# nonl4331/raytracing-rust

Measured on AMD Instinct MI355X. Metric: Msamples/s on rtweekend1.ssml 1920x1080x1024spp, higher is better.
Workload: dtype f32

## Files before the change

raytracing-rust_amd/csrc/rt_lean.h:

```cpp
#pragma once

#include "rt_vec.h"

namespace rt {


RT_FN void lean_sincos(float x, float &s, float &c)
{
	const float k = rintf(x * 0.636619746685028076172f);
	float r = fmaf(-k, 1.57079637050628662109f, x);
	r = fmaf(-k, -4.37113882867379282984e-08f, r);
	r = fmaf(-k, -1.71512451000588185479e-15f, r);
	const int q = (int)k;
	const float sk = rt_sin_kernel(r), ck = rt_cos_kernel(r);
	const bool odd = (q & 1) != 0;
	const float sv = odd ? ck : sk;
	const float cv = odd ? sk : ck;
	s = (q & 2) ? -sv : sv;
	c = ((q + 1) & 2) ? -cv : cv;
}

RT_FN float lean_acos_with(float x, float sqrt_half_one_minus_abs)
{
	const bool big = fabsf(x) > 0.5f;
	const float k = rt_asin_kernel(big ? sqrt_half_one_minus_abs : x);
	const float two_k = 2.0f * k;
	return big ? (x > 0.0f ? two_k : RT_PI - two_k) : RT_FRAC_PI_2 - k;
}
RT_FN float lean_acos(float x) { return lean_acos_with(x, sqrtf(0.5f * (1.0f - fabsf(x)))); }

RT_FN float lean_atan_unit_with(float t, float q)
{
	const bool upper = t > 0.414213567972183227539f;
	const float u = upper ? q : t;
	const float z = u * u;
	float p = fmaf(8.05374449538e-2f, z, -1.38776856032e-1f);
	p = fmaf(p, z, 1.99777106478e-1f);
	p = fmaf(p, z, -3.33329491539e-1f);
	return (upper ? RT_FRAC_PI_4 : 0.0f) + fmaf(p * z, u, u);
}
template <class DivA, class DivB> RT_FN float lean_atan2_with(float y, float x, DivA div_ratio, DivB div_octant)
{
	const float ax = fabsf(x), ay = fabsf(y);
	const bool swap = ay > ax;
	const float t = div_ratio(swap ? ax : ay, swap ? ay : ax);
	const float a = lean_atan_unit_with(t, div_octant(t - 1.0f, t + 1.0f));
	float r = swap ? RT_FRAC_PI_2 - a : a;
	r = (ax == ay) ? RT_FRAC_PI_4 : r;
	r = (ax == 0.0f && ay == 0.0f) ? 0.0f : r;
	if (rt_f32_bits(x) & 0x80000000u)
		r = RT_PI - r;
	r = (rt_f32_bits(y) & 0x80000000u) ? -r : r;
	return (x != x || y != y) ? x + y : r;
}
RT_FN float lean_atan2_portable(float y, float x)
{
	return lean_atan2_with(y, x, [](float n, float d) { return n / d; }, [](float n, float d) { return n / d; });
}

RT_FN float div_by_verified(float x, float c, float rc)
{
	const float q0 = x * rc;
	const float e = fmaf(-c, q0, x);
	return fmaf(e, rc, q0);
}
constexpr float kRcpPi = 1.0f / RT_PI, kRcpTau = 1.0f / RT_TAU;

#if defined(__HIP_DEVICE_COMPILE__)

__device__ __forceinline__ float lean_rcp_refined(float d)
{
	const float r0 = __builtin_amdgcn_rcpf(d);
	const float e = __builtin_fmaf(-d, r0, 1.0f);
	return __builtin_fmaf(e, r0, r0);
}
__device__ __forceinline__ float lean_div_core(float n, float d, float r1)
{
	const float q0 = n * r1;
	const float e1 = __builtin_fmaf(-d, q0, n);
	const float q1 = __builtin_fmaf(e1, r1, q0);
	const float e2 = __builtin_fmaf(-d, q1, n);
	return __builtin_fmaf(e2, r1, q1);
}
__device__ __forceinline__ float lean_div(float n, float d) { return lean_div_core(n, d, lean_rcp_refined(d)); }
__device__ __forceinline__ float lean_div_fix(float n, float d)
{
	return __builtin_amdgcn_div_fixupf(lean_div_core(n, d, lean_rcp_refined(d)), d, n);
}
__device__ __forceinline__ float lean_inv(float d)
{
	const float r1 = lean_rcp_refined(d);
	const float e1 = __builtin_fmaf(-d, r1, 1.0f);
	const float q1 = __builtin_fmaf(e1, r1, r1);
	const float e2 = __builtin_fmaf(-d, q1, 1.0f);
	return __builtin_fmaf(e2, r1, q1);
}
__device__ __forceinline__ V3 lean_div3(V3 v, float d)
{
	const float r1 = lean_rcp_refined(d);
	return V3{lean_div_core(v.x, d, r1), lean_div_core(v.y, d, r1), lean_div_core(v.z, d, r1)};
}
__device__ __forceinline__ V3 lean_div3_fix(V3 v, float d)
{
	const float r1 = lean_rcp_refined(d);
	return V3{__builtin_amdgcn_div_fixupf(lean_div_core(v.x, d, r1), d, v.x), __builtin_amdgcn_div_fixupf(lean_div_core(v.y, d, r1), d, v.y),
	          __builtin_amdgcn_div_fixupf(lean_div_core(v.z, d, r1), d, v.z)};
}

__device__ __forceinline__ float lean_sqrt(float x)
{
	const float s = __builtin_amdgcn_sqrtf(x);
	const float s_dn = __uint_as_float(__float_as_uint(s) - 1u);
	const float s_up = __uint_as_float(__float_as_uint(s) + 1u);
	const float r_dn = __builtin_fmaf(-s_dn, s, x);
	const float r_up = __builtin_fmaf(-s_up, s, x);
	float r = (r_dn <= 0.0f) ? s_dn : s;
	r = (r_up > 0.0f) ? s_up : r;
	return r;
}
constexpr float kLeanSqrtMin = 0x1p-96f;

__device__ __forceinline__ float lean_atan2(float y, float x)
{
	return lean_atan2_with(y, x, [](float n, float d) { return n / d; }, [](float n, float d) { return lean_div_fix(n, d); });
}
__device__ __forceinline__ float lean_acos_dev(float x) { return lean_acos_with(x, lean_sqrt(0.5f * (1.0f - fabsf(x)))); }
#else
RT_FN float lean_rcp_refined(float d) { return 1.0f / d; }
RT_FN float lean_div_core(float n, float d, float) { return n / d; }
RT_FN float lean_div(float n, float d) { return n / d; }
RT_FN float lean_div_fix(float n, float d) { return n / d; }
RT_FN float lean_inv(float d) { return 1.0f / d; }
RT_FN V3 lean_div3(V3 v, float d) { return v / d; }
RT_FN V3 lean_div3_fix(V3 v, float d) { return v / d; }
RT_FN float lean_sqrt(float x) { return sqrtf(x); }
constexpr float kLeanSqrtMin = 0x1p-96f;
RT_FN float lean_atan2(float y, float x) { return lean_atan2_portable(y, x); }
RT_FN float lean_acos_dev(float x) { return lean_acos(x); }
#endif

}
```

raytracing-rust_amd/csrc/rt_render.hip:

```cpp
#include "rt_shade.h"

namespace rt {

enum : int {
	PH_GEN = 0,
	PH_NODE = 1,
	PH_LEAF = 2,
	PH_SHADE = 3,
	PH_LIGHT = 4,
	PH_SCATTER = 5,
	PH_NARROW = 6,
	PH_COUNT = 7,
	PH_NEED_PIXEL = 7,
	PH_DONE = 8,
	PH_WALK = 9
};

#ifndef RT_PQ_SPLIT
#define RT_PQ_SPLIT 1
#endif
#ifndef RT_LIGHT_PHASE_THRESHOLD
#define RT_LIGHT_PHASE_THRESHOLD 48
#endif
constexpr uint32_t kLightPhaseThreshold = RT_LIGHT_PHASE_THRESHOLD;
// ... 114 lines not shown
	unsigned long long *rays_shot;
	uint32_t *work_counter;
	uint32_t *stack_ovf;
	DevPairScene pair;
};
#if defined(__HIP_DEVICE_COMPILE__)
typedef const __attribute__((address_space(4))) RenderArgs *KArgs;
#else
typedef const RenderArgs *KArgs;
#endif

template <int METHOD, bool PRUNE, bool FINE, bool SKY_LDS, class F, bool XCHG = false>
__global__ __launch_bounds__((KernelShape<F, FINE, XCHG>::max_block), (KernelShape<F, FINE, XCHG>::waves_per_simd)) void render_kernel(const RenderArgs args_by_value)
{
	extern __shared__ __align__(16) uint32_t lds[];
	const uint32_t lane = threadIdx.x & 63u;
	const uint32_t wave = threadIdx.x >> 6;

	(void)args_by_value;
#if defined(__HIP_DEVICE_COMPILE__)
	const KArgs K = (KArgs)__builtin_amdgcn_kernarg_segment_ptr();
	auto kargs = [&]() -> KArgs {
		KArgs k = K;
		asm volatile("" : "+s"(k));
		return k;
	};
#else
	const KArgs K = &args_by_value;
	auto kargs = [&]() -> KArgs { return K; };
#endif
	DevPairScene PS = {};
	auto load_pair_scene = [&]() {
		if constexpr (F::pair) {
			const KArgs k = kargs();
#pragma unroll
			for (int i = 0; i < 3; ++i) {
				PS.c0min[i] = k->pair.c0min[i]; PS.c0max[i] = k->pair.c0max[i];
				PS.c1min[i] = k->pair.c1min[i]; PS.c1max[i] = k->pair.c1max[i];
				PS.sky_c1[i] = k->pair.sky_c1[i]; PS.sky_c2[i] = k->pair.sky_c2[i];
			}
			PS.slot0 = k->pair.slot0; PS.slot1 = k->pair.slot1; PS.rank0 = k->pair.rank0; PS.rank1 = k->pair.rank1;
#pragma unroll
			for (int i = 0; i < 4; ++i) {
				PS.sphere[0][i] = k->pair.sphere[0][i]; PS.sphere[1][i] = k->pair.sphere[1][i];
				PS.lambert[0][i] = k->pair.lambert[0][i]; PS.lambert[1][i] = k->pair.lambert[1][i];
			}
			PS.inv_radius[0] = k->pair.inv_radius[0]; PS.inv_radius[1] = k->pair.inv_radius[1];
			PS.sky_param = k->pair.sky_param;
			PS.sky_tex_type = k->pair.sky_tex_type;
		}
	};
	const DevScene S_global = K->S;
	const DevRenderParams P = K->P;
	uint32_t *const stack_ovf = K->stack_ovf;
	DevScene S = S_global;

	SkyTables T;
	uint32_t sky_words = 0;
	if (SKY_LDS) {
		const uint32_t n_rows = S.sky.res_y * (S.sky.res_x + 1u);
		const uint32_t n_all = n_rows + S.sky.res_y + 1u;
		float *lds_sky = reinterpret_cast<float *>(lds);
		for (uint32_t i = threadIdx.x; i < n_all; i += blockDim.x)
			lds_sky[i] = S.sky.row_cdf[i];
		__syncthreads();
		sky_words = (n_all + 3u) & ~3u;
		const uint32_t guide_words = (S.sky.res_y + 1u) * S.sky.guide_k / 4u;
		uint32_t *lds_guide = lds + sky_words;
		const uint32_t *src_guide = reinterpret_cast<const uint32_t *>(S.sky.guide);
		for (uint32_t i = threadIdx.x; i < guide_words; i += blockDim.x)
			lds_guide[i] = src_guide[i];
		__syncthreads();
		T.row_cdf = lds_sky;
		T.marginal_cdf = lds_sky + n_rows;
		T.guide = reinterpret_cast<const uint8_t *>(lds_guide);
		sky_words += guide_words;
	} else {
		T.row_cdf = S.sky.row_cdf;
		T.marginal_cdf = S.sky.marginal_cdf;
		T.guide = S.sky.guide;
	}
	T.guide_k = S.sky.guide_k;
	T.inv_res = reinterpret_cast<KWords>(&K->S.sky.inv_res_ok);
	uint32_t blob_words = 0;
	if (!FINE && P.scene_in_lds) {
		uint32_t *lds_blob = lds + sky_words;
		blob_words = S.blob_bytes / 4u;
		for (uint32_t i = threadIdx.x; i < blob_words; i += blockDim.x)
			lds_blob[i] = S.blob[i];
		__syncthreads();
		const char *b = reinterpret_cast<const char *>(lds_blob);
		S.nodes = reinterpret_cast<const DevNode *>(b + S.off_nodes);
		S.prims = reinterpret_cast<const DevPrim *>(b + S.off_prims);
		S.shade = reinterpret_cast<const DevShade *>(b + S.off_shade);
		S.prim_rank = reinterpret_cast<const uint32_t *>(b + S.off_rank);
		S.materials = reinterpret_cast<const DevMaterial *>(b + S.off_materials);
		S.textures = reinterpret_cast<const DevTexture *>(b + S.off_textures);
		S.lights = reinterpret_cast<const uint32_t *>(b + S.off_lights);
		S.big_leaves = reinterpret_cast<const uint2 *>(b + S.off_big_leaves);
	}
	StackMem SM;
	SM.cap = P.stack_cap;
	SM.ovf_depth = P.stack_ovf_depth;
	SM.ovf = stack_ovf;
	SM.region = lds + sky_words + blob_words;
	uint32_t *stk = SM.region + wave * (P.stack_cap * kStackStride) + lane;
	uint32_t *pool = nullptr;
	if constexpr (XCHG) {
		pool = lds + (((uint32_t)(SM.region - lds) + (blockDim.x >> 6) * (P.stack_cap * kStackStride) + 3u) & ~3u);
		if (FINE) {
			if (threadIdx.x < kXchgFineHdr)
				pool[threadIdx.x] = threadIdx.x == 3u ? kXchgShaderWaves : (threadIdx.x == 4u ? (blockDim.x >> 6) - kXchgShaderWaves : 0u);
		} else if (threadIdx.x < 4u) {
			pool[threadIdx.x] = 0u;
		}
		__syncthreads();
	}

#ifdef RT_STATS
	unsigned long long st_iters[2] = {0, 0}, st_active[2] = {0, 0}, st_gen = 0, st_hist[8] = {};
	unsigned long long st_sect[16] = {}, st_mark = wall_clock64();
	unsigned long long st_fine_clock[PH_COUNT + 1] = {};
	unsigned long long st_fine_iters[PH_COUNT] = {}, st_fine_active[PH_COUNT] = {};
#endif
	const bool sky_samplable = sky_can_sample(S);
	constexpr int known_path = F::known_materials ? kMatLambertian : kMatRead;

	int ph = PH_NEED_PIXEL;
	rt_rng rng = {1u, 2u, 3u, 4u};
	Ray ray;
	ray.o = ray.d = ray.inv = ray.shear = v3s(0.0f);
	uint32_t node = kRefDone;
	int sp = 0;
	float best_t = 0.0f;
	uint32_t best_prim = kNoPrim;
	bool any_hit = false;
	V3 thr = v3s(1.0f), outp = v3s(0.0f), mean = v3s(0.0f), wo = v3s(0.0f);
	Hit hit;
	hit.t = 0.0f;
	hit.point = hit.error = hit.normal = v3s(0.0f);
	hit.err_dot = 0.0f;
	hit.uvx = hit.uvy = 0.0f;
	hit.has_uv = hit.out = false;
	uint32_t mat = 0;
	uint32_t depth = 0, sample_local = 0, out_index = 0, pixel_index = 0, px = 0, py = 0;
	uint32_t chunk_begin = 0, chunk_n = P.spp;
	uint32_t ray_count = 0;
	unsigned long long rays_total = 0;
	bool primary = true;
	struct LightCtx {
		V3 l_wi;
		float pdf_multiplier;
		float t_limit;
		uint32_t skip;
		bool have_shadow, shadow_is_sky;
	};
	LightCtx PL;
	PL.l_wi = v3s(0.0f);
	PL.pdf_multiplier = 1.0f;
	PL.t_limit = 0.0f;
	PL.skip = kNoPrim;
	PL.have_shadow = PL.shadow_is_sky = false;

	auto begin_walk = [&](bool shadow) {
		any_hit = shadow;
		best_t = 0.0f;
		best_prim = kNoPrim;
		sp = 0;
		if (!FINE) {
			ph = PH_NODE;
			return;
		}
		if (XCHG) {
			ph = PH_WALK;
			return;
		}
		if (root_box_misses(S, ray)) {
			node = kRefDone;
			ph = shadow ? PH_SCATTER : PH_SHADE;
		} else if (S.narrow_only != 0u || !ray_is_regular(ray)) {
			ph = PH_NARROW;
		} else {
			node = S.root4_ref;
			ph = ref_is_leaf(node) ? PH_LEAF : PH_NODE;
		}
	};
	auto start_walk = [&]() {
		sp = 0;
		if (root_box_misses(S, ray)) {
			node = kRefDone;
			ph = any_hit ? PH_SCATTER : PH_SHADE;
		} else if (S.narrow_only != 0u || !ray_is_regular(ray)) {
			ph = PH_NARROW;
		} else {
			node = S.root4_ref;
			ph = ref_is_leaf(node) ? PH_LEAF : PH_NODE;
		}
	};
	auto after_step = [&]() {
		if (node == kRefDone)
			ph = any_hit ? PH_SCATTER : PH_SHADE;
		else
			ph = ref_is_leaf(node) ? PH_LEAF : PH_NODE;
	};
	auto finalize = [&](bool filter) {
		V3 c = outp;
		if (filter && (contains_nan(c) || !is_finite_any(c)))
			c = v3s(0.0f);
		if (P.sample_split > 1u) {
			mean.x += c.x;
			mean.y += c.y;
			mean.z += c.z;
		} else {
			const float i_f = (float)(sample_local + 1u);
			mean.x += (c.x - mean.x) / i_f;
			mean.y += (c.y - mean.y) / i_f;
			mean.z += (c.z - mean.z) / i_f;
		}
		rays_total += ray_count;
		sample_local += 1;
		if (sample_local == chunk_n) {
			float *const out = kargs()->out;
			out[3u * (size_t)out_index + 0u] = mean.x;
			out[3u * (size_t)out_index + 1u] = mean.y;
			out[3u * (size_t)out_index + 2u] = mean.z;
			ph = PH_NEED_PIXEL;
		} else {
			ph = PH_GEN;
		}
	};

	auto do_gen = [&]() {
		const KArgs k = kargs();
		const uint64_t seed = ((uint64_t)k->P.seed_hi << 32) | k->P.seed_lo;
		const uint64_t sample_begin = ((uint64_t)k->P.sample_begin_hi << 32) | k->P.sample_begin_lo;
		const V3 cam_o = v3(k->cam.origin[0], k->cam.origin[1], k->cam.origin[2]);
		const V3 cam_ll = v3(k->cam.lower_left[0], k->cam.lower_left[1], k->cam.lower_left[2]);
		const V3 cam_h = v3(k->cam.horizontal[0], k->cam.horizontal[1], k->cam.horizontal[2]);
		const V3 cam_v = v3(k->cam.vertical[0], k->cam.vertical[1], k->cam.vertical[2]);
		const uint32_t w1 = here_(k->P.width - 1u), h1 = here_(k->P.height - 1u);
		rt_rng_seed(&rng, seed, (uint64_t)pixel_index, sample_begin + chunk_begin + sample_local);
		RT_SECTION(15);
		const float jx = rt_rng_range_f32(&rng, 0.0f, 1.0f) + (float)px, jy = rt_rng_range_f32(&rng, 0.0f, 1.0f) + (float)py;
		float u, v;
		if (here_(k->P.w1h1_ok) != 0u) {
// ... 64 lines not shown
					else
						take = false;
					if (take) {
						best_t = t;
						best_prim = slot;
					}
				}
			}
		}
		if (occluded) {
			best_prim = 0u;
			node = kRefDone;
		} else if (sp == 0) {
			node = kRefDone;
		} else {
			--sp;
			node = SM.ovf_depth == 0u ? stack_load<false>(SM, stk, sp) : stack_load<true>(SM, stk, sp);
		}
		after_step();
	
	};

	auto do_shade = [&](auto arm_tag) {
		constexpr int arm = decltype(arm_tag)::value;
		const uint32_t prim = best_prim;
		bool finish = false;
		bool filter = true;
		Hit nh;
		uint32_t nmat;
		if (prim != kNoPrim)
			make_hit<F>(S, prim, ray, best_t, nh, nmat, PS);
		else
			make_sky_hit_lean<F>(S, nh, nmat);
		const int known_new = F::known_materials ? (prim == kNoPrim ? kMatEmit : kMatLambertian) : kMatRead;

		if (METHOD == 0) {
			ray_count += 1;
			const V3 wo_n = ray.d;
			const V3 emission = emission_of_hit<F>(S, PS, nmat, prim == kNoPrim, nh, wo_n);
			const bool exit = mat_scatter_ray<F>(S, nmat, ray, nh, rng, known_new);
			if (depth == 0) {
				outp = outp + emission;
				if (exit)
					finish = true;
			}
			if (!finish && exit) {
				outp = outp + thr * emission;
				finish = true;
			}
			if (!finish) {
				if (!mat_is_delta<F>(S, nmat))
					thr = thr * mat_eval_over_pdf<F>(S, nmat, nh, wo_n, ray.d, known_new, PS);
				else
					thr = thr * mat_eval<F>(S, nmat, nh, wo_n, ray.d, known_new, PS);
				if (depth > P.rr_threshold) {
					const float p = component_max(thr);
					if (rt_rng_f32(&rng) > p)
						finish = true;
					else
						thr = thr / p;
				}
				if (!finish) {
					depth += 1;
					if (!(depth < P.max_depth))
						finish = true;
				}
			}
		} else if (arm == 1 || (arm == 0 && primary)) {
			wo = ray.d;
			hit = nh;
			mat = nmat;
			RT_SECTION(13);
			const V3 emission = emission_of_hit<F>(S, PS, mat, prim == kNoPrim, hit, wo);
			Ray clone = ray;
			const bool exit = mat_scatter_ray<F>(S, mat, clone, hit, rng, known_new);
			outp = outp + emission;
			RT_SECTION(14);
			if (exit) {
				finish = true;
				filter = false;
			} else {
				depth = 1;
				primary = false;
				if (!(depth < P.max_depth))
					finish = true;
			}
		} else {
			const V3 m_wi = ray.d;
			const float m_pdf = mat_scattering_pdf<F>(S, mat, hit, wo, m_wi, known_path);
			const V3 le = emission_of_hit<F>(S, PS, nmat, prim == kNoPrim, hit , m_wi);
			thr = thr * mat_eval_over_pdf<F>(S, mat, hit, wo, m_wi, known_path, PS);
			RT_SECTION(11);
			if (!is_zero(le)) {
				const bool on_light = F::lights && (prim != kNoPrim) && mat_is_light(S, nmat) && !mat_is_delta<F>(S, mat);
				if (on_light || (prim == kNoPrim && sky_samplable)) {
					const uint32_t n_l = F::lights ? S.n_lights : 0u;
					const uint32_t n_choices = sky_samplable ? n_l + 1u : n_l;
					float l_pdf;
					if (prim == kNoPrim) {
						l_pdf = div_by_count(sky_pdf(S, T, m_wi), n_choices);
					} else {
						const PrimGeom g = load_prim<F>(S, prim);
						l_pdf = div_by_count(prim_scattering_pdf<F>(g, hit.point, m_wi, nh), n_choices);
					}
					const float mis_weight = power_heuristic(m_pdf, l_pdf);
					outp = outp + thr * le * mis_weight;
				} else {
					outp = outp + thr * le;
				}
			}
			RT_SECTION(12);
			if (mat_is_light<F>(S, nmat, known_new)) {
				finish = true;
			} else {
				if (depth > P.rr_threshold) {
					const float p = component_max(thr);
					if (rt_rng_f32(&rng) > p)
						finish = true;
					else
						thr = thr / p;
				}
				if (!finish) {
					wo = m_wi;
					hit = nh;
					mat = nmat;
					depth += 1;
					if (!(depth < P.max_depth))
						finish = true;
				}
			}
		}
		if (finish)
			finalize(filter);
		else if (METHOD == 1)
			ph = PH_LIGHT;
		else
			begin_walk(false);
	
	};

	auto do_light = [&](LightCtx &L, Ray &sr) {
		ray_count += 1;
		L.have_shadow = false;
		L.shadow_is_sky = false;
		L.pdf_multiplier = 1.0f;
		L.skip = kNoPrim;
		const uint32_t samplable_len = F::lights ? S.n_lights : 0u;
		bool pick_sky = false, pick_light = false;
		uint32_t light_slot = 0;
		if (samplable_len == 0u) {
			pick_sky = sky_samplable;
		} else if (!sky_samplable) {
			L.pdf_multiplier = 1.0f / (float)samplable_len;
			light_slot = rt_rng_below(&rng, samplable_len);
			pick_light = true;
		} else {
			L.pdf_multiplier = 1.0f / (float)(samplable_len + 1u);
			light_slot = rt_rng_below(&rng, samplable_len + 1u);
			if (light_slot == samplable_len)
				pick_sky = true;
			else
				pick_light = true;
		}
		const V3 shadow_origin = hit.point + 0.0001f * hit.normal;
		PrimGeom g;
		g.type = g.material = 0u;
		g.p0 = g.p1 = g.p2 = v3s(0.0f);
		if (pick_sky) {
			L.l_wi = sky_sample(S, T, rng);
			RT_SECTION(9);
			L.t_limit = __uint_as_float(0x7FC00000u);
			L.have_shadow = true;
			L.shadow_is_sky = true;
		} else if (pick_light) {
			if (S.single_light != kNoPrim) {
				L.skip = S.single_light;
				g = load_prim_uniform<F>(&S_global.prims[L.skip]);
			} else {
				L.skip = S.lights[light_slot];
				g = load_prim<F>(S, L.skip);
			}
			L.l_wi = prim_sample_visible_from_point<F>(g, hit.point, rng);
		}
		if (pick_sky || pick_light)
			sr = ray_new<F>(shadow_origin, L.l_wi);
		if (pick_light) {
			float lt;
			if (prim_t<F>(g, sr, lt) && lt > 0.0f) {
				L.t_limit = lt;
				L.have_shadow = true;
			}
		}
		if (L.have_shadow) {
			begin_walk(true);
		} else {
			best_prim = kNoPrim;
			ph = PH_SCATTER;
		}
	
	};

	auto do_scatter = [&](LightCtx &L, Ray &sr) {
		const bool occluded = best_prim != kNoPrim;
		if (L.have_shadow && !occluded) {
			bool valid = false;
			V3 le = v3s(0.0f);
			float l_pdf = 0.0f;
			if (L.shadow_is_sky) {
				le = emission_of_hit<F>(S, PS, S.sky.material, true, hit, L.l_wi);
				l_pdf = sky_pdf(S, T, L.l_wi) * L.pdf_multiplier;
				valid = true;
			} else {
				Hit lh;
				uint32_t lm;
				PrimGeom g;
				if (S.single_light != kNoPrim) {
					g = load_prim_uniform<F>(&S_global.prims[L.skip]);
					if (!F::tri || g.type == kPrimSphere) {
						make_sphere_hit_by_reciprocal(g.p0, g.p1.x, g.p1.y, sr, L.t_limit, lh);
						lm = g.material;
					} else {
						make_hit<F>(S, L.skip, sr, L.t_limit, lh, lm);
					}
				} else {
					make_hit<F>(S, L.skip, sr, L.t_limit, lh, lm);
					g = load_prim<F>(S, L.skip);
				}
				const float p = prim_scattering_pdf<F>(g, hit.point, L.l_wi, lh);
				if (p > 0.0f) {
					le = mat_get_emission<F>(S, lm, lh, L.l_wi);
					l_pdf = p * L.pdf_multiplier;
					valid = true;
				}
			}
			if (valid) {
				const float m_pdf = mat_scattering_pdf<F>(S, mat, hit, wo, L.l_wi, known_path);
				const float mis_weight = power_heuristic(l_pdf, m_pdf);
				outp = outp + thr * mat_eval<F>(S, mat, hit, wo, L.l_wi, known_path, PS) * mis_weight * le / l_pdf;
			}
		}
		RT_SECTION(10);
		ray.d = wo;
		if (mat_scatter_ray<F>(S, mat, ray, hit, rng, known_path))
			finalize(true);
		else
			begin_walk(false);
	
	};

	auto do_narrow = [&]() {
		if (any_hit) {
			best_prim = trace_any<F, PRUNE, true>(S, S_global, SM, ray, stk, PL.t_limit, PL.skip) ? 0u : kNoPrim;
			ph = PH_SCATTER;
		} else {
			trace_closest<F, PRUNE, true>(S, S_global, SM, ray, stk, best_t, best_prim);
			ph = PH_SHADE;
		}
		node = kRefDone;
		sp = 0;
	};

	auto walk_closest_pending = [&]() {
		if (ph == PH_NODE && !any_hit) {
			trace_closest<F, PRUNE>(S, S_global, SM, ray, stk, best_t, best_prim, PS);
			ph = PH_SHADE;
		}
	};
	auto walk_shadow_pending = [&](const LightCtx &L, const Ray &sr) {
		if (ph == PH_NODE && any_hit) {
			best_prim = trace_any<F, PRUNE>(S, S_global, SM, sr, stk, L.t_limit, L.skip, PS) ? 0u : kNoPrim;
			ph = PH_SCATTER;
		}
	};

	auto record_store = [&](uint32_t *rec) {
		uint4 *d = reinterpret_cast<uint4 *>(rec);
		const uint32_t fl = (hit.has_uv ? 1u : 0u) | (hit.out ? 2u : 0u) | (primary ? 4u : 0u) | (any_hit ? 8u : 0u) | (PL.have_shadow ? 16u : 0u) |
		                    (PL.shadow_is_sky ? 32u : 0u);
		d[0] = make_uint4(rng.s0, rng.s1, rng.s2, rng.s3);
		d[1] = make_uint4(__float_as_uint(thr.x), __float_as_uint(thr.y), __float_as_uint(thr.z), __float_as_uint(outp.x));
		d[2] = make_uint4(__float_as_uint(outp.y), __float_as_uint(outp.z), __float_as_uint(wo.x), __float_as_uint(wo.y));
		d[3] = make_uint4(__float_as_uint(wo.z), __float_as_uint(hit.t), __float_as_uint(hit.point.x), __float_as_uint(hit.point.y));
		d[4] = make_uint4(__float_as_uint(hit.point.z), __float_as_uint(hit.error.x), __float_as_uint(hit.error.y), __float_as_uint(hit.error.z));
		d[5] = make_uint4(__float_as_uint(hit.normal.x), __float_as_uint(hit.normal.y), __float_as_uint(hit.normal.z), __float_as_uint(hit.uvx));
		d[6] = make_uint4(__float_as_uint(hit.uvy), fl, mat, depth);
		d[7] = make_uint4(ray_count, __float_as_uint(mean.x), __float_as_uint(mean.y), __float_as_uint(mean.z));
		d[8] = make_uint4(sample_local, out_index, pixel_index, px);
		d[9] = make_uint4(py, chunk_begin, chunk_n, (uint32_t)ph);
		d[10] = make_uint4(__float_as_uint(ray.o.x), __float_as_uint(ray.o.y), __float_as_uint(ray.o.z), __float_as_uint(ray.d.x));
		d[11] = make_uint4(__float_as_uint(ray.d.y), __float_as_uint(ray.d.z), __float_as_uint(ray.inv.x), __float_as_uint(ray.inv.y));
		d[12] = make_uint4(__float_as_uint(ray.inv.z), __float_as_uint(ray.shear.x), __float_as_uint(ray.shear.y), __float_as_uint(ray.shear.z));
		d[13] = make_uint4(__float_as_uint(best_t), best_prim, __float_as_uint(PL.t_limit), PL.skip);
		d[14] = make_uint4(__float_as_uint(PL.l_wi.x), __float_as_uint(PL.l_wi.y), __float_as_uint(PL.l_wi.z), __float_as_uint(PL.pdf_multiplier));
// ... 492 lines not shown
		}
	}

	if constexpr (!FINE) {
		bool alive = true;
		uint32_t waited = 0;
		while (alive) {
			if (XCHG && METHOD == 1)
				exchange();
			acquire();
			const uint32_t n_light = (uint32_t)__popcll(__ballot(ph == PH_LIGHT));
			const uint32_t n_trace = (METHOD == 1 && RT_PQ_SPLIT) ? (uint32_t)__popcll(__ballot(ph == PH_GEN))
			                                                      : (uint32_t)__popcll(__ballot(ph == PH_GEN || ph == PH_NODE || ph == PH_LEAF || ph == PH_SHADE));
			constexpr bool kBodyAlways = RT_BODY_ALWAYS(KernelShape<F>::spheres_only);
			if (kBodyAlways) {
				alive = (n_light + n_trace != 0u) || __ballot(ph == PH_NEED_PIXEL) != 0ull;
				if (XCHG && METHOD == 1 && !alive)
					alive = __hip_atomic_load(&pool[1], __ATOMIC_RELAXED, __HIP_MEMORY_SCOPE_WORKGROUP) != 0u ||
					        __hip_atomic_load(&pool[2], __ATOMIC_RELAXED, __HIP_MEMORY_SCOPE_WORKGROUP) != 0u;
			}
			if (kBodyAlways || n_light + n_trace != 0u) {
				const bool run_light = (METHOD == 1) && (n_light >= kLightPhaseThreshold || n_trace == 0u || (kStarveLimit != 0u && waited >= kStarveLimit));
				waited = run_light ? 0u : waited + n_light;
	#ifdef RT_STATS
				if (lane == 0u) {
					if (!run_light) {
						st_iters[0] += 1; st_active[0] += n_trace;
						st_hist[((n_trace ? n_trace : 1u) - 1u) >> 3] += 1;
#ifndef RT_STATS_NO_HIST
						atomicAdd(&g_hist[0][n_trace], 1ull);
						atomicAdd(&g_hist[1][n_light], 1ull);
#endif
						st_gen += (unsigned long long)__popcll(__ballot(ph == PH_GEN));
					} else {
						st_iters[1] += 1; st_active[1] += n_light;
#ifndef RT_STATS_NO_HIST
						atomicAdd(&g_hist[3][n_light], 1ull);
#endif
					}
				}
	#endif
				RT_SECTION(0);
				constexpr bool kFuseRegions = METHOD == 1 && RT_PQ_SPLIT && RT_FUSE_REGIONS(KernelShape<F>::spheres_only);
				bool run_q = run_light;
				if (!run_light) {
					if (kFuseRegions) {
						if (ph == PH_GEN) {
							load_pair_scene();
							do_gen();
							RT_SECTION(1);
							walk_closest_pending();
							RT_SECTION(2);
							do_shade(std::integral_constant<int, 1>{});
						}
						RT_SECTION(3);
						const uint32_t n_light_now = (uint32_t)__popcll(__ballot(ph == PH_LIGHT));
						run_q = n_light_now >= kLightPhaseThreshold;
						if (run_q)
							waited = 0u;
	#ifdef RT_STATS
						if (run_q && lane == 0u) {
							st_iters[1] += 1; st_active[1] += n_light_now;
						}
	#endif
					} else {
						load_pair_scene();
						if (ph == PH_GEN)
							do_gen();
						RT_SECTION(1);
						walk_closest_pending();
						RT_SECTION(2);
						if (ph == PH_SHADE)
							do_shade(std::integral_constant<int, (METHOD == 1 && RT_PQ_SPLIT) ? 1 : 0>{});
						RT_SECTION(3);
					}
				}
				if (run_q) {
					LightCtx L;
					L.l_wi = v3s(0.0f);
					L.pdf_multiplier = 1.0f;
					L.t_limit = 0.0f;
					L.skip = kNoPrim;
					L.have_shadow = L.shadow_is_sky = false;
					Ray sray;
					sray.o = sray.d = sray.inv = sray.shear = v3s(0.0f);
					if (kFuseRegions) {
						if (ph == PH_LIGHT) {
							load_pair_scene();
							do_light(L, sray);
							RT_SECTION(4);
							walk_shadow_pending(L, sray);
							RT_SECTION(5);
							do_scatter(L, sray);
							RT_SECTION(6);
							if (ph == PH_NODE) {
								walk_closest_pending();
								RT_SECTION(7);
								do_shade(std::integral_constant<int, 2>{});
							}
						}
						RT_SECTION(8);
					} else {
						load_pair_scene();
						if (ph == PH_LIGHT)
							do_light(L, sray);
						RT_SECTION(4);
						walk_shadow_pending(L, sray);
						RT_SECTION(5);
						if (ph == PH_SCATTER)
							do_scatter(L, sray);
						RT_SECTION(6);
	#if RT_PQ_SPLIT
						walk_closest_pending();
						RT_SECTION(7);
						if (ph == PH_SHADE)
							do_shade(std::integral_constant<int, 2>{});
						RT_SECTION(8);
	#endif
					}
				}
	#if RT_PQ_SPLIT
				if (METHOD == 1) {
					ray.o = ray.d = ray.inv = ray.shear = v3s(0.0f);
					best_t = 0.0f;
					best_prim = kNoPrim;
					node = kRefDone;
					sp = 0;
					any_hit = false;
				}
	#endif
			} else {
				alive = __ballot(ph == PH_NEED_PIXEL) != 0ull;
				if (XCHG && METHOD == 1)
					alive = alive || __hip_atomic_load(&pool[1], __ATOMIC_RELAXED, __HIP_MEMORY_SCOPE_WORKGROUP) != 0u ||
					        __hip_atomic_load(&pool[2], __ATOMIC_RELAXED, __HIP_MEMORY_SCOPE_WORKGROUP) != 0u;
			}
		}
	}
#ifdef RT_STATS
	atomicAdd(&g_stats[20], st_lane_nodes);
	atomicAdd(&g_stats[21], st_lane_prims);
	atomicMax(&g_stats[22], st_lane_maxsp);
	if (lane == 0u) {
		for (int k = 0; k < 9; ++k)
			atomicAdd(&g_stats[40 + k], st_sect[k]);
		if (!FINE)
			for (int k = 9; k < 16; ++k)
				atomicAdd(&g_stats[40 + k], st_sect[k]);
		for (int k = 0; k < 8; ++k)
			atomicAdd(&g_stats[24 + k], st_hist[k]);
		for (int k = 0; k <= PH_COUNT; ++k)
			atomicAdd(&g_stats[50 + k], st_fine_clock[k]);
		atomicAdd(&g_stats[0], st_iters[0]); atomicAdd(&g_stats[1], st_active[0]);
		atomicAdd(&g_stats[2], st_iters[1]); atomicAdd(&g_stats[3], st_active[1]);
		atomicAdd(&g_stats[4], st_gen);
		for (int k = 0; k < PH_COUNT; ++k) {
			atomicAdd(&g_stats[5 + k], st_fine_iters[k]);
			atomicAdd(&g_stats[5 + PH_COUNT + k], st_fine_active[k]);
		}
	}
#endif
	unsigned long long *const rays_shot = K->rays_shot;
	if (rays_shot != nullptr) {
		for (int off = 32; off > 0; off >>= 1)
			rays_total += __shfl_down(rays_total, off);
		if (lane == 0u)
// ... 646 lines not shown
```

raytracing-rust_amd/csrc/rt_shade.h:

```cpp
#pragma once

#include "rt_intersect.h"

namespace rt {

__device__ __forceinline__ float sqrt_unit_(float x)
{
#if defined(__HIP_DEVICE_COMPILE__) && !defined(RT_NO_LEAN)
	return lean_sqrt(x);
#else
	return sqrtf(x);
#endif
}
__device__ __forceinline__ float div_tame_fix_(float n, float d)
{
#if defined(__HIP_DEVICE_COMPILE__) && !defined(RT_NO_LEAN)
	return lean_div_fix(n, d);
#else
	return n / d;
#endif
}

__device__ __forceinline__ float next_float(float f)
{
// ... 129 lines not shown
		return v3(t.c1[0], t.c1[1], t.c1[2]) * tt + v3(t.c2[0], t.c2[1], t.c2[2]) * (1.0f - tt);
	}
	if (!F::ctex)
		return v3s(1.0f);
	if (type == 0) {
		const float sign = rt_sinf(10.0f * point.x) * rt_sinf(10.0f * point.y) * rt_sinf(10.0f * point.z);
		return sign > 0.0f ? v3(t.c1[0], t.c1[1], t.c1[2]) : v3(t.c2[0], t.c2[1], t.c2[2]);
	}
	if (type == 2) {
		const float phi = lean_atan2(direction.y, direction.x) + kPi;
		const float theta = lean_acos_dev(direction.z);
		const float uvx = phi / (2.0f * kPi);
		const float uvy = theta / kPi;
		const uint32_t x_pixel = f32_as_index((float)t.dim_x * uvx);
		const uint32_t y_pixel = f32_as_index((float)t.dim_y * uvy);
		uint64_t index = (uint64_t)y_pixel * (t.dim_x + 1u) + x_pixel;
		const uint64_t n = (uint64_t)(t.dim_x + 1u) * (t.dim_y + 1u);
		if (index >= n)
			index = n - 1;
		const float *px = t.image + 3 * index;
		return v3(px[0], px[1], px[2]);
	}
	if (type == 4)
		return (0.5f * v3s(1.0f)) * (1.0f + perlin_noise(t, point));
	return v3s(1.0f);
}

enum : int { kMatRead = -1, kMatEmit = 0, kMatLambertian = 1 };
template <class F> __device__ __forceinline__ int mat_type_(uint32_t mat, int known)
{
	if (F::known_materials && known != kMatRead)
		return known;
	return mat_handle_type(mat);
}
__device__ __forceinline__ const DevMaterial &mat_record(const DevScene &S, uint32_t mat) { return S.materials[mat_handle_index(mat)]; }

template <class F> __device__ __forceinline__ V3 material_texture_colour(const DevScene &S, const DevMaterial &m, uint32_t mat, V3 direction, V3 point)
{
	const int type = mat_handle_tex_type(mat);
	if (type == 1)
		return v3(m.tex_c1[0], m.tex_c1[1], m.tex_c1[2]);
	if (type == 3) {
		const float tt = direction.z * 0.5f + 0.5f;
		return v3(m.tex_c1[0], m.tex_c1[1], m.tex_c1[2]) * tt + v3(m.tex_c2[0], m.tex_c2[1], m.tex_c2[2]) * (1.0f - tt);
	}
	if (!F::ctex)
		return v3s(1.0f);
	return texture_colour<F>(S, m.texture, direction, point);
}

struct LambertRec {
	V3 colour;
	float albedo;
};
template <class F> __device__ __forceinline__ LambertRec lambert_record(const DevScene &S, const DevMaterial &m, uint32_t mat, V3 direction, V3 point, const DevPairScene &ps)
{
	LambertRec L;
	if constexpr (F::known_materials) {
		const bool first = mat == ps.slot0;
		L.colour = first ? v3(ps.lambert[0][0], ps.lambert[0][1], ps.lambert[0][2]) : v3(ps.lambert[1][0], ps.lambert[1][1], ps.lambert[1][2]);
		L.albedo = first ? ps.lambert[0][3] : ps.lambert[1][3];
	} else {
		L.colour = material_texture_colour<F>(S, m, mat, direction, point);
		L.albedo = m.param;
	}
	return L;
}

__device__ __forceinline__ uint32_t here_(uint32_t uniform)
{
#if defined(__HIP_DEVICE_COMPILE__)
	asm volatile("" : "+s"(uniform));
#endif
	return uniform;
}

__device__ __forceinline__ float div_by_count(float x, uint32_t n)
{
	if ((n & (n - 1u)) == 0u && n != 0u)
		return x * __uint_as_float((127u - (uint32_t)__builtin_ctz(n)) << 23);
	return x / (float)n;
}

__device__ __forceinline__ uint32_t dist1d_sample(const float *cdf, uint32_t n, const uint8_t *guide, uint32_t guide_k, rt_rng &rng)
{
	const float num = rt_rng_f32(&rng);
	uint32_t first;
	if (guide != nullptr) {
		first = guide[(uint32_t)(num * (float)guide_k)];
		for (;;) {
			const float c0 = cdf[first > n ? n : first], c1 = cdf[first + 1u > n ? n : first + 1u];
			const bool b0 = first <= n && c0 <= num;
			const bool b1 = b0 && first + 1u <= n && c1 <= num;
			first += (b0 ? 1u : 0u) + (b1 ? 1u : 0u);
			if (!b1)
				break;
		}
	} else {
		first = 0;
		uint32_t len = n + 1;
		while (len > 0) {
			const uint32_t half = len >> 1;
			const uint32_t middle = first + half;
			if (cdf[middle] <= num) {
				first = middle + 1;
				len -= half + 1;
			} else {
				len = half;
			}
		}
	}
	const uint32_t v = first - 1u;
	return v > n - 1u ? n - 1u : v;
}

#if defined(__HIP_DEVICE_COMPILE__)
typedef const __attribute__((address_space(4))) uint32_t *KWords;
#else
typedef const uint32_t *KWords;
#endif
struct SkyTables {
	const float *row_cdf;
	const float *marginal_cdf;
	const uint8_t *guide;
	uint32_t guide_k;
	KWords inv_res;
};

__device__ __forceinline__ bool sky_can_sample(const DevScene &S) { return (S.sky.res_x | S.sky.res_y) != 0u; }

__device__ __forceinline__ float sky_pdf(const DevScene &S, const SkyTables &T, V3 wi)
{
	const float sin_theta = sqrt_unit_(1.0f - wi.z * wi.z);
	if (sin_theta <= 0.0f)
		return 0.0f;
	const float theta = lean_acos_dev(wi.z);
	float phi = lean_atan2(wi.y, wi.x);
	if (phi < 0.0f)
		phi += 2.0f * kPi;
	const float u = div_by_verified(phi, kTau, kRcpTau);
	const float v = div_by_verified(theta, kPi, kRcpPi);
	const uint32_t rx = here_(S.sky.res_x), ry = here_(S.sky.res_y);
	uint32_t ui = f32_as_index((float)rx * u);
	uint32_t vi = f32_as_index((float)ry * v);
	ui = ui > rx - 1u ? rx - 1u : ui;
	vi = vi > ry - 1u ? ry - 1u : vi;
	const float ypdf = T.marginal_cdf[vi + 1u] - T.marginal_cdf[vi];
	const float *row = T.row_cdf + (size_t)vi * (rx + 1u);
	const float xpdf = row[ui + 1u] - row[ui];
	return (float)rx * (float)ry * (ypdf * xpdf) / (sin_theta * kTau * kPi);
}

__device__ __forceinline__ V3 sky_sample(const DevScene &S, const SkyTables &T, rt_rng &rng)
{
	const uint32_t rx = here_(S.sky.res_x), ry = here_(S.sky.res_y);
	const bool guided = T.guide_k != 0u;
	const uint32_t sv = dist1d_sample(T.marginal_cdf, ry, guided ? T.guide + (size_t)ry * T.guide_k : nullptr, T.guide_k, rng);
	const uint32_t su = dist1d_sample(T.row_cdf + (size_t)sv * (rx + 1u), rx, guided ? T.guide + (size_t)sv * T.guide_k : nullptr, T.guide_k, rng);
	const float nu = next_float((float)su + rt_rng_f32(&rng)), nv = next_float((float)sv + rt_rng_f32(&rng));
	float u, v;
	KWords inv = T.inv_res;
#if defined(__HIP_DEVICE_COMPILE__)
	asm volatile("" : "+s"(inv));
#endif
	if (inv != nullptr && inv[0] != 0u) {
		u = div_by_verified(nu, (float)rx, __uint_as_float(inv[1]));
		v = div_by_verified(nv, (float)ry, __uint_as_float(inv[2]));
	} else {
		u = nu / (float)rx;
		v = nv / (float)ry;
	}
	const float phi = u * 2.0f * kPi;
	const float theta = v * kPi;
	float st, ct, sp, cp;
	lean_sincos(theta, st, ct);
	lean_sincos(phi, sp, cp);
	return v3(st * cp, st * sp, ct);
}

__device__ __forceinline__ V3 lambertian_sample(V3 normal, rt_rng &rng)
{
	const float cos_theta = sqrt_unit_(1.0f - rt_rng_f32(&rng));
	const float sin_theta = sqrt_unit_(1.0f - cos_theta * cos_theta);
	const float phi = 2.0f * kPi * rt_rng_f32(&rng);
	float sin_phi, cos_phi;
	lean_sincos(phi, sin_phi, cos_phi);
	const V3 local = v3(cos_phi * sin_theta, sin_phi * sin_theta, cos_theta);
	const Coord c = coord_from_z(normal);
	return to_coord(c, local);
}
template <bool ZSEL = false> __device__ __forceinline__ V3 lambertian_sample_(V3 normal, rt_rng &rng)
{
	const float cos_theta = sqrt_unit_(1.0f - rt_rng_f32(&rng));
	const float sin_theta = sqrt_unit_(1.0f - cos_theta * cos_theta);
	const float phi = 2.0f * kPi * rt_rng_f32(&rng);
	float sin_phi, cos_phi;
	lean_sincos(phi, sin_phi, cos_phi);
	const V3 local = v3(cos_phi * sin_theta, sin_phi * sin_theta, cos_theta);
	const Coord c = ZSEL ? coord_from_z_zsel(normal) : coord_from_z(normal);
	return to_coord(c, local);
}
__device__ __forceinline__ float tr_d(float alpha, float cos_theta)
{
	if (cos_theta <= 0.0f)
		return 0.0f;
	const float a_sq = alpha * alpha;
	const float tmp = cos_theta * cos_theta * (a_sq - 1.0f) + 1.0f;
	return a_sq / (kPi * tmp * tmp);
}
__device__ __forceinline__ float tr_g2(float alpha, V3 normal, V3 h, V3 incoming, V3 outgoing)
{
	if (dot(incoming, h) / dot(incoming, normal) <= 0.0f || dot(outgoing, h) / dot(outgoing, normal) <= 0.0f)
		return 0.0f;
	const float alpha_sq = alpha * alpha;
	const float one_minus_alpha_sq = 1.0f - alpha_sq;
	const float cos_i = dot(normal, incoming);
	const float tmp_a = alpha_sq + one_minus_alpha_sq * (cos_i * cos_i);
	const float cos_o = dot(normal, outgoing);
	const float tmp_b = alpha_sq + one_minus_alpha_sq * (cos_o * cos_o);
	return 2.0f * cos_i * cos_o / (cos_o * sqrtf(tmp_a) + cos_i * sqrtf(tmp_b));
}
__device__ __forceinline__ float tr_g1(float alpha, V3 normal, V3 h, V3 v)
{
	if (dot(v, h) / dot(v, normal) <= 0.0f)
		return 0.0f;
	const float c = dot(normal, v);
	const float alpha_sq = alpha * alpha;
	const float tmp = alpha_sq + (1.0f - alpha_sq) * (c * c);
	return 2.0f * c / (sqrtf(tmp) + c);
}
__device__ __forceinline__ float tr_vndf(float a, V3 h, V3 incoming)
{
	if (h.z < 0.0f)
		return 0.0f;
	return tr_g1(a, v3(0.0f, 0.0f, 1.0f), h, incoming) * fmax_(dot(incoming, h), 0.0f) * tr_d(a, h.z) / incoming.z;
}
__device__ inline V3 tr_sample_vndf(float a_x, float a_y, V3 incoming, rt_rng &rng)
{
	const V3 vh = normalised(v3(a_x * incoming.x, a_y * incoming.y, incoming.z));
	const float len_sq = vh.x * vh.x + vh.y * vh.y;
	const V3 basis_two = len_sq > 0.0f ? v3(-vh.y, vh.x, 0.0f) / sqrtf(len_sq) : v3(1.0f, 0.0f, 0.0f);
	const V3 basis_three = cross(vh, basis_two);
	const float r = sqrtf(rt_rng_f32(&rng));
	const float phi = kTau * rt_rng_f32(&rng);
	float sin_phi, cos_phi;
	lean_sincos(phi, sin_phi, cos_phi);
	const float tx = r * cos_phi;
// ... 266 lines not shown
```

Measured before the change: 36610.

## Reuse sampled sky cell indices to skip inverse-mapping in sky PDF

```diff
diff --git a/raytracing-rust_amd/csrc/rt_lean.h b/raytracing-rust_amd/csrc/rt_lean.h
--- a/raytracing-rust_amd/csrc/rt_lean.h
+++ b/raytracing-rust_amd/csrc/rt_lean.h
@@ -65,6 +65,17 @@
 	return fmaf(e, rc, q0);
 }
 constexpr float kRcpPi = 1.0f / RT_PI, kRcpTau = 1.0f / RT_TAU;
+
+constexpr float kSkyCellSlopeU = 0x1p-18f;
+constexpr float kSkyCellSlopeV = 0x1p-17f;
+constexpr uint32_t kSkyCellPoleShift = 8u;
+constexpr uint32_t kSkyCellMaxRes = 1200u;
+RT_FN bool sky_cell_safe(float ru, float rv, uint32_t sv, uint32_t rx, uint32_t ry)
+{
+	const float hu = 0.5f - (float)rx * kSkyCellSlopeU, hv = 0.5f - (float)ry * kSkyCellSlopeV;
+	const uint32_t k = 1u + (ry >> kSkyCellPoleShift);
+	return fabsf(ru - 0.5f) <= hu && fabsf(rv - 0.5f) <= hv && sv >= k && sv + k < ry && rx <= kSkyCellMaxRes && ry <= kSkyCellMaxRes;
+}
 
 #if defined(__HIP_DEVICE_COMPILE__)
 
diff --git a/raytracing-rust_amd/csrc/rt_render.hip b/raytracing-rust_amd/csrc/rt_render.hip
--- a/raytracing-rust_amd/csrc/rt_render.hip
+++ b/raytracing-rust_amd/csrc/rt_render.hip
@@ -220,6 +220,8 @@
 	}
 	T.guide_k = S.sky.guide_k;
 	T.inv_res = reinterpret_cast<KWords>(&K->S.sky.inv_res_ok);
+	T.kargs = reinterpret_cast<KWords>(K);
+	T.inv_res_word = (uint32_t)(offsetof(RenderArgs, S.sky.inv_res_ok) / 4u);
 	uint32_t blob_words = 0;
 	if (!FINE && P.scene_in_lds) {
 		uint32_t *lds_blob = lds + sky_words;
@@ -286,12 +288,14 @@
 	uint32_t ray_count = 0;
 	unsigned long long rays_total = 0;
 	bool primary = true;
+	constexpr bool kReuseSkyCell = F::pair;
 	struct LightCtx {
 		V3 l_wi;
 		float pdf_multiplier;
 		float t_limit;
 		uint32_t skip;
 		bool have_shadow, shadow_is_sky;
+		uint32_t known_cell;
 	};
 	LightCtx PL;
 	PL.l_wi = v3s(0.0f);
@@ -299,6 +303,7 @@
 	PL.t_limit = 0.0f;
 	PL.skip = kNoPrim;
 	PL.have_shadow = PL.shadow_is_sky = false;
+	PL.known_cell = kSkyCellUnknown;
 
 	auto begin_walk = [&](bool shadow) {
 		any_hit = shadow;
@@ -529,7 +534,7 @@
 			} else {
 				depth = 1;
 				primary = false;
-				if (!(depth < P.max_depth))
+				if (!(depth < (F::pair ? here_(P.max_depth) : P.max_depth)))
 					finish = true;
 			}
 		} else {
@@ -614,7 +619,12 @@
 		g.type = g.material = 0u;
 		g.p0 = g.p1 = g.p2 = v3s(0.0f);
 		if (pick_sky) {
-			L.l_wi = sky_sample(S, T, rng);
+			if constexpr (kReuseSkyCell) {
+				L.l_wi = sky_sample<true>(S, T, rng, L.known_cell);
+			} else {
+				uint32_t unused;
+				L.l_wi = sky_sample<false>(S, T, rng, unused);
+			}
 			RT_SECTION(9);
 			L.t_limit = __uint_as_float(0x7FC00000u);
 			L.have_shadow = true;
@@ -655,7 +665,23 @@
 			float l_pdf = 0.0f;
 			if (L.shadow_is_sky) {
 				le = emission_of_hit<F>(S, PS, S.sky.material, true, hit, L.l_wi);
-				l_pdf = sky_pdf(S, T, L.l_wi) * L.pdf_multiplier;
+				if constexpr (kReuseSkyCell) {
+					SkyCell c = sky_cell_unpack(L.known_cell);
+					const bool round_trip = __ballot(L.known_cell == kSkyCellUnknown) != 0ull;
+#ifdef RT_STATS
+					if (lane == (uint32_t)__ffsll((unsigned long long)__ballot(true)) - 1u)
+						atomicAdd(&g_stats[round_trip ? 59 : 58], 1ull);
+#endif
+					if (round_trip)
+						c = sky_cell_of(S, L.l_wi);
+					l_pdf = sky_pdf_of_cell(S, T, L.l_wi.z, c) * L.pdf_multiplier;
+				} else {
+#ifdef RT_STATS
+					if (lane == (uint32_t)__ffsll((unsigned long long)__ballot(true)) - 1u)
+						atomicAdd(&g_stats[59], 1ull);
+#endif
+					l_pdf = sky_pdf(S, T, L.l_wi) * L.pdf_multiplier;
+				}
 				valid = true;
 			} else {
 				Hit lh;
@@ -1314,6 +1340,7 @@
 					L.t_limit = 0.0f;
 					L.skip = kNoPrim;
 					L.have_shadow = L.shadow_is_sky = false;
+					L.known_cell = kSkyCellUnknown;
 					Ray sray;
 					sray.o = sray.d = sray.inv = sray.shear = v3s(0.0f);
 					if (kFuseRegions) {
diff --git a/raytracing-rust_amd/csrc/rt_shade.h b/raytracing-rust_amd/csrc/rt_shade.h
--- a/raytracing-rust_amd/csrc/rt_shade.h
+++ b/raytracing-rust_amd/csrc/rt_shade.h
@@ -235,7 +235,7 @@
 	return x / (float)n;
 }
 
-__device__ __forceinline__ uint32_t dist1d_sample(const float *cdf, uint32_t n, const uint8_t *guide, uint32_t guide_k, rt_rng &rng)
+__device__ __forceinline__ uint32_t dist1d_sample(const float *cdf, uint32_t n, const uint8_t *guide, uint32_t guide_k, rt_rng &rng, uint32_t &clamped)
 {
 	const float num = rt_rng_f32(&rng);
 	uint32_t first;
@@ -264,6 +264,7 @@
 		}
 	}
 	const uint32_t v = first - 1u;
+	clamped |= v > n - 1u ? 0xFFFFFFFFu : 0u;
 	return v > n - 1u ? n - 1u : v;
 }
 
@@ -278,15 +279,17 @@
 	const uint8_t *guide;
 	uint32_t guide_k;
 	KWords inv_res;
+	KWords kargs;
+	uint32_t inv_res_word;
 };
 
 __device__ __forceinline__ bool sky_can_sample(const DevScene &S) { return (S.sky.res_x | S.sky.res_y) != 0u; }
 
-__device__ __forceinline__ float sky_pdf(const DevScene &S, const SkyTables &T, V3 wi)
-{
-	const float sin_theta = sqrt_unit_(1.0f - wi.z * wi.z);
-	if (sin_theta <= 0.0f)
-		return 0.0f;
+struct SkyCell {
+	uint32_t u, v;
+};
+__device__ __forceinline__ SkyCell sky_cell_of(const DevScene &S, V3 wi)
+{
 	const float theta = lean_acos_dev(wi.z);
 	float phi = lean_atan2(wi.y, wi.x);
 	if (phi < 0.0f)
@@ -294,28 +297,65 @@
 	const float u = div_by_verified(phi, kTau, kRcpTau);
 	const float v = div_by_verified(theta, kPi, kRcpPi);
 	const uint32_t rx = here_(S.sky.res_x), ry = here_(S.sky.res_y);
-	uint32_t ui = f32_as_index((float)rx * u);
-	uint32_t vi = f32_as_index((float)ry * v);
-	ui = ui > rx - 1u ? rx - 1u : ui;
-	vi = vi > ry - 1u ? ry - 1u : vi;
-	const float ypdf = T.marginal_cdf[vi + 1u] - T.marginal_cdf[vi];
-	const float *row = T.row_cdf + (size_t)vi * (rx + 1u);
-	const float xpdf = row[ui + 1u] - row[ui];
+	SkyCell c;
+	c.u = f32_as_index((float)rx * u);
+	c.v = f32_as_index((float)ry * v);
+	c.u = c.u > rx - 1u ? rx - 1u : c.u;
+	c.v = c.v > ry - 1u ? ry - 1u : c.v;
+	return c;
+}
+__device__ __forceinline__ float sky_pdf_of_cell(const DevScene &S, const SkyTables &T, float wi_z, SkyCell c)
+{
+	const float sin_theta = sqrt_unit_(1.0f - wi_z * wi_z);
+	if (sin_theta <= 0.0f)
+		return 0.0f;
+	const uint32_t rx = here_(S.sky.res_x), ry = here_(S.sky.res_y);
+	const float ypdf = T.marginal_cdf[c.v + 1u] - T.marginal_cdf[c.v];
+	const float *row = T.row_cdf + (size_t)c.v * (rx + 1u);
+	const float xpdf = row[c.u + 1u] - row[c.u];
 	return (float)rx * (float)ry * (ypdf * xpdf) / (sin_theta * kTau * kPi);
 }
-
-__device__ __forceinline__ V3 sky_sample(const DevScene &S, const SkyTables &T, rt_rng &rng)
+__device__ __forceinline__ float sky_pdf(const DevScene &S, const SkyTables &T, V3 wi)
+{
+	const float sin_theta = sqrt_unit_(1.0f - wi.z * wi.z);
+	if (sin_theta <= 0.0f)
+		return 0.0f;
+	const SkyCell c = sky_cell_of(S, wi);
+	const uint32_t rx = here_(S.sky.res_x), ry = here_(S.sky.res_y);
+	const float ypdf = T.marginal_cdf[c.v + 1u] - T.marginal_cdf[c.v];
+	const float *row = T.row_cdf + (size_t)c.v * (rx + 1u);
+	const float xpdf = row[c.u + 1u] - row[c.u];
+	return (float)rx * (float)ry * (ypdf * xpdf) / (sin_theta * kTau * kPi);
+}
+
+constexpr uint32_t kSkyCellUnknown = 0xFFFFFFFFu;
+__device__ __forceinline__ SkyCell sky_cell_unpack(uint32_t known_cell)
+{
+	SkyCell c;
+	c.u = known_cell & 0xFFFFu;
+	c.v = known_cell >> 16;
+	return c;
+}
+template <bool LATE_ADDRESS> __device__ __forceinline__ V3 sky_sample(const DevScene &S, const SkyTables &T, rt_rng &rng, uint32_t &known_cell)
 {
 	const uint32_t rx = here_(S.sky.res_x), ry = here_(S.sky.res_y);
 	const bool guided = T.guide_k != 0u;
-	const uint32_t sv = dist1d_sample(T.marginal_cdf, ry, guided ? T.guide + (size_t)ry * T.guide_k : nullptr, T.guide_k, rng);
-	const uint32_t su = dist1d_sample(T.row_cdf + (size_t)sv * (rx + 1u), rx, guided ? T.guide + (size_t)sv * T.guide_k : nullptr, T.guide_k, rng);
-	const float nu = next_float((float)su + rt_rng_f32(&rng)), nv = next_float((float)sv + rt_rng_f32(&rng));
+	uint32_t clamped = 0u;
+	const uint32_t sv = dist1d_sample(T.marginal_cdf, ry, guided ? T.guide + (size_t)ry * T.guide_k : nullptr, T.guide_k, rng, clamped);
+	const uint32_t su = dist1d_sample(T.row_cdf + (size_t)sv * (rx + 1u), rx, guided ? T.guide + (size_t)sv * T.guide_k : nullptr, T.guide_k, rng, clamped);
+	const float ru = rt_rng_f32(&rng);
+	const float rv = rt_rng_f32(&rng);
+	const float nu = next_float((float)su + ru), nv = next_float((float)sv + rv);
+	static_assert(kSkyCellMaxRes < 0x10000u, "a safe cell packs into 16 + 16 bits");
+	const uint32_t unguided = here_(T.guide_k) == 0u ? kSkyCellUnknown : 0u;
+	known_cell = (sky_cell_safe(ru, rv, sv, rx, ry) ? (su | (sv << 16)) : kSkyCellUnknown) | clamped | unguided;
 	float u, v;
-	KWords inv = T.inv_res;
+	KWords inv = LATE_ADDRESS ? T.kargs : T.inv_res;
 #if defined(__HIP_DEVICE_COMPILE__)
 	asm volatile("" : "+s"(inv));
 #endif
+	if (LATE_ADDRESS)
+		inv += T.inv_res_word;
 	if (inv != nullptr && inv[0] != 0u) {
 		u = div_by_verified(nu, (float)rx, __uint_as_float(inv[1]));
 		v = div_by_verified(nv, (float)ry, __uint_as_float(inv[2]));
```

Measured after the change: 37850, median of 6. 1.03x the previous value.
